# bipul-mohanto/fovPathTracing_optixCodeLatest

Measured on AMD Instinct MI355X. Metric: Mray/s, higher is better.
Workload: dtype f32; 1 GPU; C3: Sponza-class procedural atrium, 265640 tris, 1920x1080, foveated spp fovea/mid/periphery 8/2/1, radii 148/482, gaze centre, Disney BSDF + probe NEE, depth 4, ambient probe 2.5 @ frame res; triangles=265640, width=1920, height=1080, subframe=reset to 0 every frame (as the shipped app), parallelism=single GPU, frames_in_flight=2, gather=none

## Files before the change

fovpathtracing_optixcodelatest_amd/csrc/traverse.hip:

```cpp
#include "fovpt_device.h"
#include <hip/hip_ext.h>
#include <assert.h>
#include "fovpt_pixel.h"
#include "fovpt_queue.h"
#include "fovpt_stream.h"

#ifndef FOVPT_V_WAVES
#define FOVPT_V_WAVES 8
#endif

namespace {

struct RayT {
    float ox, oy, oz, dx, dy, dz;
    float ix, iy, iz;
    float nox, noy, noz;
};

__device__ inline float safe_rcp(float d)
{
    const float a = fabsf(d) < 1e-20f ? copysignf(1e-20f, d) : d;
    return __builtin_amdgcn_rcpf(a);
}
__device__ inline void ray_setup(RayT& r, const float4& o, const float4& d)
{
    r.ox = o.x; r.oy = o.y; r.oz = o.z; r.dx = d.x; r.dy = d.y; r.dz = d.z;
    r.ix = safe_rcp(d.x); r.iy = safe_rcp(d.y); r.iz = safe_rcp(d.z);
    r.nox = -o.x * r.ix; r.noy = -o.y * r.iy; r.noz = -o.z * r.iz;
}
__device__ inline bool box_hit(const RayT& r, float lx, float ly, float lz, float hx, float hy, float hz, float tmin, float tmax, float& tn)
{
    const float ax = __builtin_fmaf(lx, r.ix, r.nox), bx = __builtin_fmaf(hx, r.ix, r.nox);
    const float ay = __builtin_fmaf(ly, r.iy, r.noy), by = __builtin_fmaf(hy, r.iy, r.noy);
    const float az = __builtin_fmaf(lz, r.iz, r.noz), bz = __builtin_fmaf(hz, r.iz, r.noz);
    const float t0 = fmaxf(fmaxf(fminf(ax, bx), fminf(ay, by)), fmaxf(fminf(az, bz), tmin));
    const float far = fminf(fminf(fmaxf(ax, bx), fmaxf(ay, by)), fmaxf(az, bz));
    const float t1 = __int_as_float(min(__float_as_int(far), __float_as_int(tmax)));
    tn = t0;
    return t0 <= t1 * 1.000001f;
}

#define TMIN 0.01f
#define TMAX 1e16f

#define TRAV_DONE ((int)0x80000000)

__device__ inline uint32_t quad_rot1(uint32_t v) { return (uint32_t)__builtin_amdgcn_mov_dpp((int)v, 0x39, 0xf, 0xf, true); }
__device__ inline uint32_t quad_rot2(uint32_t v) { return (uint32_t)__builtin_amdgcn_mov_dpp((int)v, 0x4E, 0xf, 0xf, true); }
__device__ inline uint32_t quad_rot3(uint32_t v) { return (uint32_t)__builtin_amdgcn_mov_dpp((int)v, 0x93, 0xf, 0xf, true); }

enum { ROWB = FOVPT_TQUADS * 4,
       ROWSHIFT = FOVPT_TQUADS == 16 ? 6 : FOVPT_TQUADS == 64 ? 8 : 10 };
static_assert(FOVPT_LEAF_MAX <= 4, "a leaf is tested in one quad step");
static_assert(FOVPT_TQUADS == 16 || FOVPT_TQUADS == 64 || FOVPT_TQUADS == 256, "row stride of the stack is 64, 256 or 1024 bytes");

typedef __attribute__((address_space(3))) char LdsChar;
typedef __attribute__((address_space(3))) int LdsInt;

struct QuadLane {
    uint32_t j, qshift, from_me, j32, j3;
    int miss_rows;
    __device__ inline void init()
    {
        j = threadIdx.x & 3u;
        qshift = threadIdx.x & 60u;
        from_me = 15u & ~((1u << j) - 1u);
        j32 = 32u * j; j3 = 3u * j;
        miss_rows = (int)(j + 1u) * ROWB;
    }
};
struct QuadTrav {
    int cur;
    LdsChar* top;
    float lim;
    float bt, bu, bv; uint32_t bpos, bprim;
#if FOVPT_V_STEPSTAT
    uint32_t steps;
    uint32_t n0;
#endif
    __device__ inline void start(int* stack, const QuadLane& q)
    {
        if (q.j == 0) stack[0] = TRAV_DONE;
        top = (LdsChar*)(LdsInt*)stack + ROWB;
        cur = 0; lim = TMAX;
        bt = INFINITY; bu = 0.f; bv = 0.f; bpos = 0xffffffffu; bprim = 0xffffffffu;
    }
};

#if FOVPT_V_STEPSTAT
__device__ inline void stepstat(unsigned long long* diag)
{
    const unsigned long long ex = __builtin_amdgcn_ballot_w64(true);
    if ((threadIdx.x & 63u) == (uint32_t)__builtin_ctzll(ex)) { atomicAdd(diag + 0, 1ull); atomicAdd(diag + 1, (unsigned long long)(__builtin_popcountll(ex) >> 2)); }
}
#define STEPSTAT(d) stepstat(d)
#else
#define STEPSTAT(d)
#endif

#define FOVPT_TOPN 5
__shared__ float4 s_top[FOVPT_TOPN * 8];

template <bool ANY_HIT>
__device__ inline void node_finish(const RayT& r, const QuadLane& q, QuadTrav& T, const float4& a, const float4& b)
{
    const int code = __float_as_int(b.z);
    float t;
    const bool h = box_hit(r, a.x, a.y, a.z, a.w, b.x, b.y, TMIN, T.lim, t);
    const uint32_t m4 = (uint32_t)(__builtin_amdgcn_ballot_w64(h) >> q.qshift) & 15u;
    int Hm1;
    asm("v_bcnt_u32_b32 %0, %1, -1" : "=v"(Hm1) : "v"(m4));
#if FOVPT_V_STEPSTAT
    if (m4 == 0u) T.n0++;
#endif
    int row;
    if (ANY_HIT) {
        row = ((__builtin_popcount(m4 & q.from_me) - 1) << ROWSHIFT) + (h ? 0 : q.miss_rows);
    } else {
        uint32_t key;
        asm("v_and_or_b32 %0, %1, -4, %2" : "=v"(key) : "v"(h ? __float_as_uint(t) : 0u), "v"(__float_as_uint(b.w)));
        const int lt = ((int)(quad_rot1(key) - key) >> 31) + ((int)(quad_rot2(key) - key) >> 31) + ((int)(quad_rot3(key) - key) >> 31);
        row = (lt << ROWSHIFT) + 3 * ROWB;
    }
    *(LdsInt*)(T.top + row) = code;
    T.top += Hm1 * ROWB;
    __builtin_amdgcn_wave_barrier();
    T.cur = *(const LdsInt*)T.top;
}

template <bool ANY_HIT, bool TOP = false>
__device__ inline void node_step(const SceneView& sc, const RayT& r, const QuadLane& q, QuadTrav& T)
{
    const float4* np = (const float4*)((const char*)sc.nodes + (((uint32_t)T.cur << 7) | q.j32));
    float4 a, b;
    if (TOP) {
        typedef __attribute__((address_space(3))) float LdsFloat;
        const LdsFloat* lp = (const LdsFloat*)((const LdsChar*)(LdsFloat*)(float*)s_top + (((uint32_t)T.cur << 7) | q.j32));
        a = make_float4(lp[0], lp[1], lp[2], lp[3]); b = make_float4(lp[4], lp[5], lp[6], lp[7]);
    } else { a = np[0]; b = np[1]; }
    node_finish<ANY_HIT>(r, q, T, a, b);
}

template <bool ANY_HIT>
__device__ inline bool leaf_finish(const RayT& r, const QuadLane& q, QuadTrav& T, const TriRec& R, uint32_t tri16)
{
    const V3 d = v3(r.dx, r.dy, r.dz);
    const V3 e1 = v3(R.e1x, R.e1y, R.e1z), e2 = v3(R.e2x, R.e2y, R.e2z);
    const V3 p = cross(d, e2);
    const float det = dot(e1, p);
    const float inv = 1.0f / det;
    const V3 s = v3(r.ox, r.oy, r.oz) - v3(R.v0x, R.v0y, R.v0z);
    const float u = dot(s, p) * inv;
    const V3 qq = cross(s, e1);
    const float v = dot(d, qq) * inv;
    const float t = dot(e2, qq) * inv;
    const bool ok = (u >= 0.0f) & (v >= 0.0f) & (u + v <= 1.0f) & (t > TMIN) & (t < TMAX);
    if (ANY_HIT) {
        if ((uint32_t)(__builtin_amdgcn_ballot_w64(ok & (det > 0.0f)) >> q.qshift) & 15u) return true;
    } else {
        const bool better = ok & ((t < T.bt) | ((t == T.bt) & (R.prim < T.bprim)));
        T.bt = better ? t : T.bt; T.bu = better ? u : T.bu; T.bv = better ? v : T.bv;
        T.bpos = better ? tri16 : T.bpos; T.bprim = better ? R.prim : T.bprim;
        uint32_t m = __float_as_uint(T.bt);
        m = min(m, quad_rot2(m));
        m = min(m, quad_rot1(m));
        T.lim = fminf(TMAX, __uint_as_float(m) * 1.000001f);
    }
    T.top -= ROWB;
    T.cur = *(const LdsInt*)T.top;
    return false;
}

template <bool ANY_HIT>
__device__ inline bool mixed_step(const SceneView& sc, const RayT& r, const QuadLane& q, QuadTrav& T, unsigned long long* diag)
{
    const bool at_node = T.cur >= 0;
    const uint32_t lcode = (uint32_t)~T.cur;
    const uint32_t tri16 = (lcode >> 3) + (q.j <= (lcode & 7u) ? q.j3 : 0u);
    const uint32_t off = at_node ? (((uint32_t)T.cur << 7) | q.j32) : sc.tri_off + (tri16 << 4);
    const float4* p = (const float4*)((const char*)sc.nodes + off);
    const float4 x0 = p[0], x1 = p[1], x2 = p[2];
    if (at_node) {
        STEPSTAT(diag);
        node_finish<ANY_HIT>(r, q, T, x0, x1);
        return false;
    }
    STEPSTAT(diag + 2);
    TriRec R;
    R.v0x = x0.x; R.v0y = x0.y; R.v0z = x0.z; R.e1x = x0.w;
    R.e1y = x1.x; R.e1z = x1.y; R.e2x = x1.z; R.e2y = x1.w;
    R.e2z = x2.x; R.prim = __float_as_uint(x2.y); R.mesh = __float_as_uint(x2.z); R.pad = 0;
    return leaf_finish<ANY_HIT>(r, q, T, R, tri16);
}

__device__ inline void store_hit(const PathState& ps, uint32_t ph, const QuadTrav& T)
{
    uint32_t mt = __float_as_uint(T.bt);
    mt = min(mt, quad_rot2(mt));
    mt = min(mt, quad_rot1(mt));
    const bool cand = __float_as_uint(T.bt) == mt;
    uint32_t mp = cand ? T.bprim : 0xffffffffu;
    mp = min(mp, quad_rot2(mp));
    mp = min(mp, quad_rot1(mp));
    if (cand && T.bprim == mp) st_stream<FOVPT_STREAM_HIT>(ps.hit + ph, make_float4(T.bt, T.bu, T.bv, __uint_as_float(T.bpos)));
}
__device__ inline void store_shadow(const PathState& ps, const ShadowQueue& sq, uint32_t ph, uint32_t slot, uint32_t target, bool occluded)
{
    const float4 val = occluded ? ld_stream<FOVPT_STREAM_SHADOWQ>(sq.val_occ + ph) : ld_stream<FOVPT_STREAM_SHADOWQ>(sq.val_vis + ph);
    float4* cell = target == 0xffffffffu ? ps.alpha + slot : ps.rad + ((size_t)slot * ps.stride + target);
    st_stream<FOVPT_STREAM_CELLS>(cell, make_float4(val.x, val.y, val.z, 0.f));
}

#ifndef FOVPT_VOTE_A
#define FOVPT_VOTE_A 2
#endif
#ifndef FOVPT_VOTE_B
#define FOVPT_VOTE_B 1
#endif
#ifndef FOVPT_VOTE_C
#define FOVPT_VOTE_C 1
#endif
__device__ inline bool vote_leaf(uint32_t na, uint32_t nn)
{
    return (na - nn) * (uint32_t)FOVPT_VOTE_A >= nn * (uint32_t)FOVPT_VOTE_B + 4u * (uint32_t)FOVPT_VOTE_C;
}

__device__ inline void traverse_quad(const SceneView& sc, const RayT& r, int* __restrict__ stack , const QuadLane& q,
                              QuadTrav& T, unsigned long long* diag)
{
    T.start(stack, q);
#if FOVPT_V_STEPSTAT
    uint32_t my_nodes = 0u, my_leaves = 0u;
    T.n0 = 0u;
#define RAYSTAT(x) (x)++
#else
#define RAYSTAT(x)
#endif
    if (sc.num_nodes >= FOVPT_TOPN) {
        STEPSTAT(diag);
        node_step<false, true>(sc, r, q, T);
        RAYSTAT(my_nodes);
        if (T.cur >= 0 && T.cur < FOVPT_TOPN) { STEPSTAT(diag); node_step<false, true>(sc, r, q, T); RAYSTAT(my_nodes); }
    }
    while (T.cur != TRAV_DONE) {
        const uint32_t na = (uint32_t)__builtin_popcountll(__builtin_amdgcn_ballot_w64(true));
        while (T.cur >= 0) {
            STEPSTAT(diag);
            node_step<false>(sc, r, q, T);
            RAYSTAT(my_nodes);
            const uint32_t nn = (uint32_t)__builtin_popcountll(__builtin_amdgcn_ballot_w64(T.cur >= 0));
            if (vote_leaf(na, nn)) break;
        }
        if (T.cur != TRAV_DONE) {
#if FOVPT_V_STEPSTAT
            if (T.cur >= 0) my_nodes++; else my_leaves++;
#endif
            mixed_step<false>(sc, r, q, T, diag);
        }
    }
#if FOVPT_V_STEPSTAT
    T.steps = min(my_nodes, 4095u) | (min(my_leaves, 255u) << 12) | (min(T.n0, 63u) << 20);
#endif
#undef RAYSTAT
}

#ifndef FOVPT_REFILL
#define FOVPT_REFILL 6
#endif
__device__ inline void traverse_shadow_pool(const SceneView& sc, const PathState& ps, const ShadowQueue& sq, const ShardMap& map, uint32_t cap,
                                            uint32_t first, uint32_t end, int* __restrict__ stack, const QuadLane& q, unsigned long long* diag)
{
    QuadTrav T;
    T.start(stack, q);
    T.cur = TRAV_DONE;
    RayT r = {};
    uint32_t ph = 0;
    bool pending = false, occluded = false;
    uint32_t next = first;
    for (;;) {
        const unsigned long long idle = __builtin_amdgcn_ballot_w64(T.cur == TRAV_DONE);
        const uint32_t n_idle = (uint32_t)__builtin_popcountll(idle) >> 2;
        if (n_idle == 16u || (n_idle >= (uint32_t)FOVPT_REFILL && next < end)) {
            if (T.cur == TRAV_DONE) {
                if (pending && q.j == 0) store_shadow(ps, sq, ph, __float_as_uint(ld_stream<FOVPT_STREAM_SHADOWQ>(&sq.o[ph].w)),
                                                          __float_as_uint(ld_stream<FOVPT_STREAM_SHADOWQ>(&sq.d[ph].w)), occluded);
                pending = false;
                const uint32_t rank = (__builtin_amdgcn_mbcnt_hi((uint32_t)(idle >> 32), __builtin_amdgcn_mbcnt_lo((uint32_t)idle, 0u)) - q.j) >> 2;
                const uint32_t idx = next + rank;
                if (idx < end) {
                    ph = map.phys16(idx, next, cap);
                    ray_setup(r, ld_stream<FOVPT_STREAM_SHADOWQ>(sq.o + ph), ld_stream<FOVPT_STREAM_SHADOWQ>(sq.d + ph));
                    T.start(stack, q);
                    pending = true; occluded = false;
                }
            }
            next = min(end, next + n_idle);
            if (n_idle == 16u && __builtin_amdgcn_ballot_w64(T.cur != TRAV_DONE) == 0ull) return;
        }
        const uint32_t na = (uint32_t)__builtin_popcountll(__builtin_amdgcn_ballot_w64(T.cur != TRAV_DONE));
        while (T.cur >= 0) {
            STEPSTAT(diag);
            node_step<true>(sc, r, q, T);
            const uint32_t nn = (uint32_t)__builtin_popcountll(__builtin_amdgcn_ballot_w64(T.cur >= 0));
            if (vote_leaf(na, nn)) break;
        }
        if (T.cur != TRAV_DONE) {
            if (mixed_step<true>(sc, r, q, T, diag)) { occluded = true; T.cur = TRAV_DONE; }
        }
    }
}

template <int MODE>
__global__ __launch_bounds__(FOVPT_TBLOCK, FOVPT_V_WAVES) void k_traverse(SceneView sc, PathState ps, RayQueue queue, ShadowQueue sq,
                                                                         uint32_t cap, Counters* __restrict__ cnt, int it_closest, int it_shadow, uint32_t sel)
{
    __shared__ int s_stack[(FOVPT_STACK + 4) * FOVPT_TQUADS];
    static_assert(MODE == 0 || MODE == 1, "closest hit or occlusion");
    const int it = MODE == 0 ? it_closest : it_shadow;
    ShardMap map;
    map.load(cnt, MODE == 0 ? FOVPT_CNT_Q(it >= 0 ? it : 0) : FOVPT_CNT_SQ(it >= 0 ? it : 0), sel, cap);
    const uint32_t n_cl = (MODE == 0 && it >= 0) ? map.total() : 0u;
    const uint32_t n_sh = (MODE == 1 && it >= 0) ? map.total() : 0u;
    if (blockIdx.x == 0 && threadIdx.x == 0) {
        if (n_cl) atomicAdd(&cnt->stat_radiance, (unsigned long long)n_cl);
        if (n_sh) atomicAdd(&cnt->stat_shadow, (unsigned long long)n_sh);
        if (MODE == 0 && it == 0) atomicAdd(&cnt->stat_paths, (unsigned long long)n_cl);
    }
    QuadLane q;
    q.init();
    int* stack = s_stack + (threadIdx.x >> 2);
    if (MODE == 0 && sc.num_nodes >= FOVPT_TOPN) {
        for (uint32_t k = threadIdx.x; k < FOVPT_TOPN * 8u; k += FOVPT_TBLOCK) s_top[k] = ((const float4*)sc.nodes)[k];
        __syncthreads();
    }
    if (n_sh) {
        const uint32_t nwaves = gridDim.x * (FOVPT_TBLOCK / 64), wave = blockIdx.x * (FOVPT_TBLOCK / 64) + (threadIdx.x >> 6);
        const uint32_t per = (n_sh + nwaves - 1u) / nwaves, first = min(n_sh, wave * per);
        traverse_shadow_pool(sc, ps, sq, map, cap, first, min(n_sh, first + per), stack, q, cnt->diag[1]);
    }
    const uint32_t quads = gridDim.x * FOVPT_TQUADS;
    for (uint32_t i = blockIdx.x * FOVPT_TQUADS + (threadIdx.x >> 2); i < n_cl; i += quads) {
        const uint32_t i0 = __builtin_amdgcn_readfirstlane(i - ((threadIdx.x & 63u) >> 2));
        RayT r;
        QuadTrav T;
        const uint32_t ph = map.phys16(i, i0, cap);
        const float4 o = ld_stream<FOVPT_STREAM_RAYQ>(queue.o + ph), d = ld_stream<FOVPT_STREAM_RAYQ>(queue.d + ph);
        ray_setup(r, o, d);
        traverse_quad(sc, r, stack, q, T, cnt->diag[0]);
        store_hit(ps, ph, T);
#if FOVPT_V_STEPSTAT
        if (q.j == 0) ((uint32_t*)&queue.d[ph])[3] = T.steps;
#endif
    }
}

}

void fovpt_launch_traverse(hipStream_t st, SceneView sc, PathState ps, RayQueue queue, ShadowQueue sq, uint32_t cap,
                           Counters* cnt, int it_closest, int it_shadow, int grid, hipEvent_t done, uint32_t sel)
{
    assert(it_closest < 0 || it_shadow < 0);
    int blocks = grid * FOVPT_BLOCK / FOVPT_TBLOCK > 0 ? grid * FOVPT_BLOCK / FOVPT_TBLOCK : 1;
    if (it_shadow < 0) {
        const unsigned long long rounds = ((sel ? 4ull : 8ull) * cap + FOVPT_TQUADS - 1) / FOVPT_TQUADS;
        if ((unsigned long long)blocks > rounds) blocks = (int)((rounds + FOVPT_SHARDS - 1) / FOVPT_SHARDS * FOVPT_SHARDS);
    }
    auto kernel = it_shadow < 0 ? k_traverse<0> : k_traverse<1>;
    if (done) hipExtLaunchKernelGGL(kernel, dim3(blocks), dim3(FOVPT_TBLOCK), 0, st, nullptr, done, 0, sc, ps, queue, sq, cap, cnt, it_closest, it_shadow, sel);
    else hipLaunchKernelGGL(kernel, dim3(blocks), dim3(FOVPT_TBLOCK), 0, st, sc, ps, queue, sq, cap, cnt, it_closest, it_shadow, sel);
}
```

Baseline: 4729 Mray/s.

## Split shadow-ray record loads across quad lanes and use LDS top nodes in shadow traversal

In the shadow pool, each lane of a quad now loads one of the four record float4s (origin, direction, visible value, occluded value). Origin and direction are broadcast within the quad with DPP moves, and the lane that holds the matching value does the final store. This replaces redundant per-lane loads and a later reload for the store. Shadow traversal also now copies the top BVH nodes into LDS and runs the first one or two node steps from that LDS copy right after a refill. The changes touch load distribution, the exit condition (now based on the pending flag) and the prologue of the shadow kernel. They add DPP traffic and an LDS copy plus barrier in shadow launches.

```diff
diff --git a/fovpathtracing_optixcodelatest_amd/csrc/traverse.hip b/fovpathtracing_optixcodelatest_amd/csrc/traverse.hip
--- a/fovpathtracing_optixcodelatest_amd/csrc/traverse.hip
+++ b/fovpathtracing_optixcodelatest_amd/csrc/traverse.hip
@@ -48,6 +48,14 @@
 __device__ inline uint32_t quad_rot1(uint32_t v) { return (uint32_t)__builtin_amdgcn_mov_dpp((int)v, 0x39, 0xf, 0xf, true); }
 __device__ inline uint32_t quad_rot2(uint32_t v) { return (uint32_t)__builtin_amdgcn_mov_dpp((int)v, 0x4E, 0xf, 0xf, true); }
 __device__ inline uint32_t quad_rot3(uint32_t v) { return (uint32_t)__builtin_amdgcn_mov_dpp((int)v, 0x93, 0xf, 0xf, true); }
+__device__ inline float quad_from0(float v) { return __int_as_float(__builtin_amdgcn_mov_dpp(__float_as_int(v), 0x00, 0xf, 0xf, true)); }
+__device__ inline float quad_from1(float v) { return __int_as_float(__builtin_amdgcn_mov_dpp(__float_as_int(v), 0x55, 0xf, 0xf, true)); }
+
+__device__ inline void quad_ray(const float4& v, float4& o, float4& d)
+{
+    o = make_float4(quad_from0(v.x), quad_from0(v.y), quad_from0(v.z), quad_from0(v.w));
+    d = make_float4(quad_from1(v.x), quad_from1(v.y), quad_from1(v.z), quad_from1(v.w));
+}
 
 enum { ROWB = FOVPT_TQUADS * 4,
        ROWSHIFT = FOVPT_TQUADS == 16 ? 6 : FOVPT_TQUADS == 64 ? 8 : 10 };
@@ -204,13 +212,6 @@
     mp = min(mp, quad_rot1(mp));
     if (cand && T.bprim == mp) st_stream<FOVPT_STREAM_HIT>(ps.hit + ph, make_float4(T.bt, T.bu, T.bv, __uint_as_float(T.bpos)));
 }
-__device__ inline void store_shadow(const PathState& ps, const ShadowQueue& sq, uint32_t ph, uint32_t slot, uint32_t target, bool occluded)
-{
-    const float4 val = occluded ? ld_stream<FOVPT_STREAM_SHADOWQ>(sq.val_occ + ph) : ld_stream<FOVPT_STREAM_SHADOWQ>(sq.val_vis + ph);
-    float4* cell = target == 0xffffffffu ? ps.alpha + slot : ps.rad + ((size_t)slot * ps.stride + target);
-    st_stream<FOVPT_STREAM_CELLS>(cell, make_float4(val.x, val.y, val.z, 0.f));
-}
-
 #ifndef FOVPT_VOTE_A
 #define FOVPT_VOTE_A 2
 #endif
@@ -274,28 +275,41 @@
     T.start(stack, q);
     T.cur = TRAV_DONE;
     RayT r = {};
-    uint32_t ph = 0;
     bool pending = false, occluded = false;
     uint32_t next = first;
+    uint32_t slot = 0, target = 0;
+    float vx = 0.f, vy = 0.f, vz = 0.f;
+    const float4* const mine = q.j == 0 ? sq.o : q.j == 1 ? sq.d : q.j == 2 ? sq.val_vis : sq.val_occ;
     for (;;) {
         const unsigned long long idle = __builtin_amdgcn_ballot_w64(T.cur == TRAV_DONE);
         const uint32_t n_idle = (uint32_t)__builtin_popcountll(idle) >> 2;
         if (n_idle == 16u || (n_idle >= (uint32_t)FOVPT_REFILL && next < end)) {
             if (T.cur == TRAV_DONE) {
-                if (pending && q.j == 0) store_shadow(ps, sq, ph, __float_as_uint(ld_stream<FOVPT_STREAM_SHADOWQ>(&sq.o[ph].w)),
-                                                          __float_as_uint(ld_stream<FOVPT_STREAM_SHADOWQ>(&sq.d[ph].w)), occluded);
+                if (pending && q.j == (occluded ? 3u : 2u)) {
+                    float4* cell = target == 0xffffffffu ? ps.alpha + slot : ps.rad + ((size_t)slot * ps.stride + target);
+                    st_stream<FOVPT_STREAM_CELLS>(cell, make_float4(vx, vy, vz, 0.f));
+                }
                 pending = false;
                 const uint32_t rank = (__builtin_amdgcn_mbcnt_hi((uint32_t)(idle >> 32), __builtin_amdgcn_mbcnt_lo((uint32_t)idle, 0u)) - q.j) >> 2;
                 const uint32_t idx = next + rank;
                 if (idx < end) {
-                    ph = map.phys16(idx, next, cap);
-                    ray_setup(r, ld_stream<FOVPT_STREAM_SHADOWQ>(sq.o + ph), ld_stream<FOVPT_STREAM_SHADOWQ>(sq.d + ph));
+                    const float4 v = ld_stream<FOVPT_STREAM_SHADOWQ>(mine + map.phys16(idx, next, cap));
+                    float4 o, d;
+                    quad_ray(v, o, d);
+                    slot = __float_as_uint(o.w); target = __float_as_uint(d.w);
+                    vx = v.x; vy = v.y; vz = v.z;
+                    ray_setup(r, o, d);
                     T.start(stack, q);
                     pending = true; occluded = false;
+                    if (sc.num_nodes >= FOVPT_TOPN) {
+                        STEPSTAT(diag);
+                        node_step<true, true>(sc, r, q, T);
+                        if (T.cur >= 0 && T.cur < FOVPT_TOPN) { STEPSTAT(diag); node_step<true, true>(sc, r, q, T); }
+                    }
                 }
             }
             next = min(end, next + n_idle);
-            if (n_idle == 16u && __builtin_amdgcn_ballot_w64(T.cur != TRAV_DONE) == 0ull) return;
+            if (n_idle == 16u && __builtin_amdgcn_ballot_w64(pending) == 0ull) return;
         }
         const uint32_t na = (uint32_t)__builtin_popcountll(__builtin_amdgcn_ballot_w64(T.cur != TRAV_DONE));
         while (T.cur >= 0) {
@@ -329,7 +343,7 @@
     QuadLane q;
     q.init();
     int* stack = s_stack + (threadIdx.x >> 2);
-    if (MODE == 0 && sc.num_nodes >= FOVPT_TOPN) {
+    if (sc.num_nodes >= FOVPT_TOPN) {
         for (uint32_t k = threadIdx.x; k < FOVPT_TOPN * 8u; k += FOVPT_TBLOCK) s_top[k] = ((const float4*)sc.nodes)[k];
         __syncthreads();
     }
```

New measurement: 4695 Mray/s. Within noise of the previous version (-0.7%).
